# Chrixtar/latentsplat

Hardware: AMD Instinct MI355X
Metric: rendered target views/sec at 256x256, ~300k Gaussians (forward); fwd+bwd ms/view in `fwdbwd` (higher is better)
Workload: dtype f32; 1 GPU; BASELINE configs[1]: 300000 latent Gaussians (4-ch features + opacity), 256x256, forward render; 16 views of one scene per step per GPU; gaussians=300000, parallelism=replicas x1 (one scene per rank, no data-path collective)

## Files before the change

latentsplat_amd/csrc/lsr_key_emit.h:

```cpp
#pragma once
#include "lsr_blend.h"
#include "lsr_tile_scan.h"

namespace lsr {

struct TileRect { int x0, y0, x1, y1; };

__device__ __forceinline__ void count_pairs(uint32_t *hist, int gx, TileRect r, uint32_t span, bool skip_none) {
    if (skip_none) reached_rect(span, r.x0, r.y0, r.x1, r.y1);
    for (int y = r.y0; y < r.y1; ++y)
        for (int x = r.x0; x < r.x1; ++x) atomicAdd(&hist[y * gx + x], 1u);
}

__device__ __forceinline__ void store_bin_record(char *binrec, int narrow, size_t o, bool ok, const TileRect &r, float tz, uint32_t span) {
    const float out_depth = ok ? tz : 0.0f;
    if (narrow) {
        BinRec br;
        br.rect = ok ? ((uint32_t)r.x0 | ((uint32_t)r.y0 << 8) | ((uint32_t)r.x1 << 16) | ((uint32_t)r.y1 << 24)) : 0u;
        br.depth = out_depth; br.span = span;
        ((BinRec *)binrec)[o] = br;
    } else {
        BinRecWide br;
        br.rect = ok ? make_ushort4((unsigned short)r.x0, (unsigned short)r.y0, (unsigned short)r.x1, (unsigned short)r.y1)
                     : make_ushort4(0, 0, 0, 0);
        br.depth = out_depth; br.span = span;
        ((BinRecWide *)binrec)[o] = br;
    }
}

template <int THREADS>
__device__ __forceinline__ void flush_counts(const uint32_t *s_hist, uint32_t *tile_count, int n) {
    __syncthreads();
    for (int t = threadIdx.x; t < n; t += THREADS) {
        const uint32_t c = s_hist[t];
        if (c) atomicAdd(&tile_count[t], c);
    }
}

template <int THREADS>
__device__ __forceinline__ void reserve_segments(const uint32_t *s_hist, uint32_t *s_first, uint32_t *tile_count, int n) {
    __syncthreads();
    for (int t0 = threadIdx.x; t0 < n; t0 += 4 * THREADS) {
        uint32_t c[4], first[4] = {0u, 0u, 0u, 0u};
#pragma unroll
        for (int k = 0; k < 4; ++k) { const int t = t0 + k * THREADS; c[k] = t < n ? s_hist[t] : 0u; }
#pragma unroll
        for (int k = 0; k < 4; ++k) {
            const int t = t0 + k * THREADS;
            if (c[k]) first[k] = __hip_atomic_fetch_add(&tile_count[t], c[k], __ATOMIC_RELAXED, __HIP_MEMORY_SCOPE_AGENT);
        }
#pragma unroll
        for (int k = 0; k < 4; ++k) { const int t = t0 + k * THREADS; if (t < n) s_first[t] = first[k]; }
    }
    __syncthreads();
}

struct KeyBuckets {
    uint32_t *delta;
    uint64_t *key;
    uint32_t *pos;
    uint32_t buf;
    __device__ __forceinline__ KeyBuckets(void *area, size_t bytes, int T) {
        const int kbase = (T * 4 + 7) & ~7;
        delta = (uint32_t *)area;
        key = (uint64_t *)((char *)area + kbase);
        buf = (uint32_t)((bytes - kbase) / 12);
        pos = (uint32_t *)((char *)area + kbase + (size_t)buf * 8);
    }
};

template <int THREADS, int N>
__device__ __forceinline__ void emit_view_keys(uint32_t *cur, const uint32_t *first, const KeyBuckets &kb, const SegOut &seg,
                                               uint32_t seg_view, int T, int gx, bool skip_none,
                                               const uint3 (&br)[N], const int (&index)[N], const bool (&valid)[N]) {
    __shared__ uint32_t s_scanw[THREADS / LSR_WAVE];
    const int tpt = (T + THREADS - 1) / THREADS;
    uint32_t cnt[4], mine = 0;
#pragma unroll
    for (int k = 0; k < 4; ++k) {
        const int t = (int)threadIdx.x * tpt + k;
        cnt[k] = (k < tpt && t < T) ? cur[t] : 0u;
        mine += cnt[k];
    }
    uint32_t n_v;
    uint32_t off = block_exclusive_scan<THREADS>(mine, s_scanw, n_v);
#pragma unroll
    for (int k = 0; k < 4; ++k) {
        const int t = (int)threadIdx.x * tpt + k;
        if (k < tpt && t < T) { cur[t] = off; kb.delta[t] = first[t] - off; off += cnt[k]; }
    }
    __syncthreads();
    const uint32_t cap = seg.cap, seg0 = seg_view * (uint32_t)T;
#pragma unroll
    for (int it = 0; it < N; ++it) {
        const uint32_t rc = valid[it] ? br[it].x : 0u;
        const int x0 = rc & 0xff, y0 = (rc >> 8) & 0xff, x1 = (rc >> 16) & 0xff, y1 = rc >> 24;
        const uint64_t key = ((uint64_t)br[it].y << 32) | ((uint32_t)index[it] << seg.key_shift);
        const uint32_t sp = br[it].z;
        int ex0 = x0, ey0 = y0, ex1 = x1, ey1 = y1;
        if (skip_none) reached_rect(sp, ex0, ey0, ex1, ey1);
        for (int y = ey0; y < ey1; ++y)
            for (int x = ex0; x < ex1; ++x) {
                const int t = y * gx + x;
                const uint32_t code = seg.key_shift ? span_code(sp, x - x0, y - y0) : 0u;
                const uint32_t slot = atomicAdd(&cur[t], 1u);
                const uint32_t pos = (seg0 + (uint32_t)t) * cap + min(slot + kb.delta[t], cap - 1u);
                if (slot < kb.buf) { kb.key[slot] = key | code; kb.pos[slot] = pos; }
                else seg.keys[pos] = key | code;
            }
    }
    __syncthreads();
    const uint32_t nflush = min(n_v, kb.buf);
    for (uint32_t j = threadIdx.x; j < nflush; j += THREADS) seg.keys[kb.pos[j]] = kb.key[j];
    __syncthreads();
}

template <int THREADS>
__device__ __forceinline__ void folded_tile_scan(const FoldedScan &fs, uint32_t *header, const uint32_t *tile_count, int N,
                                                 uint32_t *s_counts, TileScanShared<THREADS> &s_scan) {
    __shared__ uint32_t s_last;
    asm volatile("s_waitcnt vmcnt(0)" ::: "memory");
    __syncthreads();
    if (threadIdx.x == 0) {
        const uint32_t arrived = __hip_atomic_fetch_add(&header[kHdrPreDone], 1u, __ATOMIC_RELAXED, __HIP_MEMORY_SCOPE_AGENT);
        s_last = arrived == gridDim.x * gridDim.y - 1u;
    }
    __syncthreads();
    if (!s_last) return;
    for (int i0 = threadIdx.x; i0 < N; i0 += 4 * THREADS) {
        uint32_t c[4];
#pragma unroll
        for (int k = 0; k < 4; ++k)
            c[k] = __hip_atomic_load(&tile_count[min(i0 + k * THREADS, N - 1)], __ATOMIC_RELAXED, __HIP_MEMORY_SCOPE_AGENT);
#pragma unroll
        for (int k = 0; k < 4; ++k)
            if (i0 + k * THREADS < N) s_counts[i0 + k * THREADS] = c[k];
    }
    __syncthreads();
    tile_scan_block<THREADS, 0, false>(s_counts, fs.tile_start, header, HostMirror{fs.host_words, fs.host_seq},
                                       fs.tile_order, N, fs.capacity, s_scan);
}

}
```

latentsplat_amd/csrc/preprocess.hip:

```cpp
#include <algorithm>

#include "lsr_blend.h"
#include "lsr_depth.h"
#include "lsr_key_emit.h"
#include "lsr_project.h"

namespace lsr {

typedef const float __attribute__((address_space(4))) *kfloat_ptr;

constexpr int kPreThreads = 256;
static_assert(kPreThreads == kPreThreadsScan, "the folded tile scan is sized for this workgroup");
constexpr int kPreItems = 8;

template <int COLOR_MODE, bool LDS_HIST, int VB, bool FMA, bool SEG, bool AA = false>
__global__ void __launch_bounds__(kPreThreads, 6)
k_preprocess(lsr_dims d, lsr_inputs in, float *__restrict__ rec, int RF, char *__restrict__ binrec, int narrow,
             int32_t *__restrict__ radii, uint32_t *__restrict__ tile_count, uint32_t *header, FoldedScan fs, int kItems, SegOut seg) {
    static_assert(!SEG || LDS_HIST, "the key emission reserves its slots from the LDS histogram");
    extern __shared__ uint32_t s_hist[];
    constexpr int kRecRow = kPreThreads + 4;
    __shared__ float4 s_rec[kRecRow * 4];
    static_assert(sizeof(float4) * kRecRow * 4 >= sizeof(uint32_t) * kFoldTiles, "the folded tile scan stages its counts here");
    const bool staged = RF == 16;
    const int v0 = blockIdx.y * VB;
    const int G = d.num_gaussians;
    const int gx = (d.width + LSR_TILE - 1) / LSR_TILE, gy = (d.height + LSR_TILE - 1) / LSR_TILE;
    const int T = gx * gy;
    __shared__ float2 s_focal[VB];
    if (threadIdx.x < VB && v0 + (int)threadIdx.x < d.num_views) {
        const float *vw = in.views + (size_t)(v0 + threadIdx.x) * LSR_VIEW_FLOATS;
        s_focal[threadIdx.x] = make_float2(d.width / (2.0f * vw[35]), d.height / (2.0f * vw[36]));
    }
    if (LDS_HIST)
        for (int t = threadIdx.x; t < VB * T; t += kPreThreads) s_hist[t] = 0;
    __syncthreads();
    const int ce = d.cov_elems;
    const size_t sl = (size_t)input_slice(d, v0);
    const float *means = in.means3D + sl * d.vs_means;
    const float *covs = in.cov3D + sl * d.vs_cov;
    const float *opac = in.opacities + sl * d.vs_opac;
    constexpr int coff = COLOR_MODE == LSR_COLOR_NONE ? 0 : 3;
    const bool direct_feat = d.feat_mode == LSR_FEAT_DIRECT;
    const bool skip_none = reached_only(d);

    const int base = blockIdx.x * (kPreThreads * kItems);
#pragma unroll 1
    for (int it = 0; it < kItems; ++it) {
        const int chunk0 = base + it * kPreThreads;
        if (chunk0 >= G) break;
        const int i = chunk0 + threadIdx.x;
        const bool in_range = i < G;
        const size_t ii = in_range ? (size_t)i : 0;
        const float q0 = means[3 * ii], q1 = means[3 * ii + 1], q2 = means[3 * ii + 2];
        const float *c6 = covs + (size_t)ce * ii;
        const float r0 = c6[0], r1 = c6[1], r2 = c6[2];
        const float r3 = c6[ce == 9 ? 4 : 3], r4 = c6[ce == 9 ? 5 : 4], r5 = c6[ce == 9 ? 8 : 5];
        const float opacity = opac[ii];
        float pay_in[3] = {0.0f, 0.0f, 0.0f};
        if (COLOR_MODE == LSR_COLOR_PRECOMP) {
            const float *cp = in.color + sl * d.vs_color + 3 * ii;
            pay_in[0] = cp[0]; pay_in[1] = cp[1]; pay_in[2] = cp[2];
        }
        const float *fp = in.features + sl * d.vs_feat + ii * d.feat_channels;
        auto payload = [&](int c4) {
            float w[4];
#pragma unroll
            for (int k = 0; k < 4; ++k) {
                const int c = 4 * c4 + k;
                w[k] = c < coff ? pay_in[c < 3 ? c : 0]
                                : ((direct_feat && c - coff < d.feat_channels) ? fp[c - coff] : 0.0f);
            }
            return make_float4(w[0], w[1], w[2], w[3]);
        };
        float4 pay0 = make_float4(0, 0, 0, 0), pay1 = make_float4(0, 0, 0, 0);
        if (staged) { pay0 = payload(0); pay1 = payload(1); }
        asm volatile("" :: "v"(q0), "v"(q1), "v"(q2), "v"(r0), "v"(r1), "v"(r2), "v"(r3), "v"(r4), "v"(r5), "v"(opacity),
                     "v"(pay0.x), "v"(pay0.y), "v"(pay0.z), "v"(pay0.w), "v"(pay1.x), "v"(pay1.y), "v"(pay1.z), "v"(pay1.w));

#pragma unroll 1
        for (int vb = 0; vb < VB; ++vb) {
            const int v = v0 + vb;
            if (v >= d.num_views) break;
            const kfloat_ptr vw = (kfloat_ptr)(in.views + (size_t)v * LSR_VIEW_FLOATS);
            float vm[16], pm[16];
#pragma unroll
            for (int k = 0; k < 16; ++k) { vm[k] = vw[k]; pm[k] = vw[16 + k]; }
            const float tanfovx = vw[35], tanfovy = vw[36];
            const float focal_x = s_focal[vb].x, focal_y = s_focal[vb].y;
            const float limx = 1.3f * tanfovx, limy = 1.3f * tanfovy;
            const float scale = vw[40], scale2 = scale * scale;
            const size_t o = (size_t)v * G + ii;
            const float p0 = q0 * scale, p1 = q1 * scale, p2 = q2 * scale;
            const float s0 = r0 * scale2, s1 = r1 * scale2, s2 = r2 * scale2;
            const float s3 = r3 * scale2, s4 = r4 * scale2, s5 = r5 * scale2;
            const Projected pj = project_gaussian<FMA, AA>(vm, pm, limx, limy, focal_x, focal_y, p0, p1, p2, s0, s1, s2, s3, s4, s5,
                                                       d.width, d.height, gx, gy, in_range);
            const bool ok = pj.ok;
            const float px = pj.px, py = pj.py, conic_a = pj.conic_a, conic_b = pj.conic_b, conic_c = pj.conic_c, tz = pj.tz;
            const float my_radius = pj.radius;
            const float rec_opacity = AA ? opacity * pj.rho : opacity;
            const TileRect rect{pj.rminx, pj.rminy, pj.rmaxx, pj.rmaxy};

            float zpay = tz;
            if (vw[41] != 0.0f) zpay = depth_mode_payload((int)vw[41], tz, scale, vw[42], vw[43]);
            const float4 rr0 = make_float4(px, py, conic_a, conic_b);
            const float4 rr1 = make_float4(conic_c, rec_opacity, ok ? zpay : -1.0f, 0.0f);
            const uint32_t span = ok ? footprint_cells(px, py, conic_a, conic_b, conic_c, rec_opacity, rect.x0, rect.y0) : kSpanNone;
            if (ok) {
                if (!staged) {
                    float4 *R = (float4 *)(rec + o * (size_t)RF);
                    R[0] = rr0; R[1] = rr1;
                    for (int c4 = 0; c4 < (RF - 8) / 4; ++c4) R[2 + c4] = payload(c4);
                }
                count_pairs(LDS_HIST ? s_hist + vb * T : tile_count + (size_t)v * T, gx, rect, span, skip_none);
            }
            if (in_range) {
                radii[o] = ok ? (int32_t)my_radius : 0;
                store_bin_record(binrec, narrow, o, ok, rect, tz, span);
            }
            if (staged) {
                s_rec[0 * kRecRow + threadIdx.x] = rr0;
                s_rec[1 * kRecRow + threadIdx.x] = rr1;
                s_rec[2 * kRecRow + threadIdx.x] = pay0;
                s_rec[3 * kRecRow + threadIdx.x] = pay1;
                __syncthreads();
                float4 *dst = (float4 *)(rec + ((size_t)v * G + chunk0) * 16);
                const int nrec = G - chunk0 < kPreThreads ? G - chunk0 : kPreThreads;
#pragma unroll
                for (int k = 0; k < 4; ++k) {
                    const int idx = k * kPreThreads + threadIdx.x;
                    if (idx < nrec * 4 && s_rec[kRecRow + (idx >> 2)].z >= 0.0f) dst[idx] = s_rec[(idx & 3) * kRecRow + (idx >> 2)];
                }
                __syncthreads();
            }
        }
    }
    const int n_valid = min(VB, d.num_views - v0) * T;
    if (LDS_HIST && !SEG) flush_counts<kPreThreads>(s_hist, tile_count + (size_t)v0 * T, n_valid);
    if (SEG) {
        uint32_t *s_first = s_hist + VB * T;
        reserve_segments<kPreThreads>(s_hist, s_first, tile_count + (size_t)v0 * T, n_valid);
        constexpr int KI = kPreItems / VB;
        const KeyBuckets kb(s_rec, sizeof(s_rec), T);
#pragma unroll 1
        for (int vb = 0; vb < VB; ++vb) {
            const int v = v0 + vb;
            if (v >= d.num_views) break;
            uint3 br[KI];
            int index[KI];
            bool valid[KI];
#pragma unroll
            for (int it = 0; it < KI; ++it) {
                const int i = min(base + min(it, kItems - 1) * kPreThreads + (int)threadIdx.x, G - 1);
                br[it] = *(const uint3 *)(binrec + ((size_t)v * G + (size_t)i) * sizeof(BinRec));
                index[it] = base + it * kPreThreads + (int)threadIdx.x;
                valid[it] = it < kItems && index[it] < G;
            }
            emit_view_keys<kPreThreads, KI>(s_hist + vb * T, s_first + vb * T, kb, seg, (uint32_t)v, T, gx, skip_none, br, index, valid);
        }
    }
    if (fs.enabled) {
        __shared__ TileScanShared<kPreThreads> s_scan;
        folded_tile_scan<kPreThreads>(fs, header, tile_count, d.num_views * T, (uint32_t *)s_rec, s_scan);
    }
}

__global__ void __launch_bounds__(256) k_clear16(uint4 *p, size_t n) {
    for (size_t i = (size_t)blockIdx.x * 256 + threadIdx.x; i < n; i += (size_t)gridDim.x * 256) p[i] = make_uint4(0u, 0u, 0u, 0u);
}
hipError_t launch_clear(void *ptr, size_t bytes, hipStream_t s) {
    const size_t n16 = bytes / 16;
    if (n16 == 0) return hipSuccess;
    const size_t blocks = (n16 + 255) / 256;
    hipLaunchKernelGGL(k_clear16, dim3((unsigned)(blocks < 65536 ? blocks : 65536)), dim3(256), 0, s, (uint4 *)ptr, n16);
    return hipGetLastError();
}

hipError_t launch_preprocess(const lsr_dims &d, const lsr_inputs &in, char *geom, int32_t *radii, const FoldedScan &fs_in,
                             bool seg_mode, hipStream_t s) {
    const GeomLayout L = geom_layout(d);
    const int T = (int)num_tiles(d);
    {
        hipError_t e = launch_clear(geom + L.header, L.tile_start - L.header, s);
        if (e != hipSuccess) return e;
    }
    if (d.num_gaussians == 0) return hipSuccess;
    const bool shared = d.vs_means == 0 && d.vs_cov == 0 && d.vs_opac == 0 && (d.color_mode != LSR_COLOR_PRECOMP || d.vs_color == 0) &&
                        (d.feat_channels == 0 || d.vs_feat == 0);
    const int span = shared ? d.num_views : (d.views_per_group > 1 ? d.views_per_group : 1);
    int vb = (span % 4 == 0 || (shared && span >= 4)) ? 4 : ((span % 2 == 0 || (shared && span >= 2)) ? 2 : 1);
    if (const int forced_vb = env_int("LSR_PRE_VB", 0)) vb = std::min(vb, forced_vb >= 4 ? 4 : (forced_vb >= 2 ? 2 : 1));
    const int64_t yblocks = (d.num_views + vb - 1) / vb;
    const int64_t fill = ((int64_t)d.num_gaussians * yblocks + (int64_t)kPreThreads * 2 * device_cus() - 1) / ((int64_t)kPreThreads * 2 * device_cus());
    const int pre_items = seg_mode ? std::min(kPreItems, std::max(1, env_int("LSR_PRE_ITEMS", kPreItems))) : std::max(1, env_int("LSR_PRE_ITEMS", kPreItems));
    const int items = (int)std::max<int64_t>(1, std::min<int64_t>(std::max(1, pre_items / vb), fill));
    dim3 grid((d.num_gaussians + kPreThreads * items - 1) / (kPreThreads * items), (unsigned)yblocks);
    float *rec = (float *)(geom + L.rec);
    char *binrec = geom + L.bin;
    const int narrow = narrow_bins(d) ? 1 : 0;
    const int RF = L.rec_floats;
    uint32_t *tc = (uint32_t *)(geom + L.tile_count);
    FoldedScan fs = fs_in;
    fs.tile_start = (uint32_t *)(geom + L.tile_start); fs.tile_order = (uint32_t *)(geom + L.tile_order);
    const bool lds = (size_t)T * vb <= 4096;
    const size_t shm = lds ? (size_t)T * vb * 4 * (seg_mode ? 2 : 1) : 0;
    const bool fma = projection_contraction();
    SegOut so{nullptr, 0u, index_packing(d).key_shift};
    if (seg_mode) {
        if (!lds || !narrow || L.seg_cap == 0) return hipErrorInvalidValue;
        so.keys = (uint64_t *)(geom + L.seg_keys); so.cap = L.seg_cap;
    }
    const bool aa = (d.forward_flags & LSR_FWD_ANTIALIAS) != 0;
#define LSR_PRE5(CM, LH, VBV, FM, SG, AAV) hipLaunchKernelGGL((k_preprocess<CM, LH, VBV, FM, SG, AAV>), grid, dim3(kPreThreads), shm, s, d, in, rec, RF, binrec, narrow, radii, tc, (uint32_t *)(geom + L.header), fs, items, so)
#define LSR_PRE4(CM, LH, VBV, FM, SG) do { if (aa) LSR_PRE5(CM, LH, VBV, FM, SG, true); else LSR_PRE5(CM, LH, VBV, FM, SG, false); } while (0)
#define LSR_PRE3(CM, LH, VBV, FM) do { if (LH && seg_mode) LSR_PRE4(CM, LH, VBV, FM, LH); else LSR_PRE4(CM, LH, VBV, FM, false); } while (0)
#define LSR_PRE2(CM, LH, VBV) do { if (fma) LSR_PRE3(CM, LH, VBV, true); else LSR_PRE3(CM, LH, VBV, false); } while (0)
#define LSR_PRE(CM)                                                                              \
    do {                                                                                         \
        if (lds) { if (vb == 4) LSR_PRE2(CM, true, 4); else if (vb == 2) LSR_PRE2(CM, true, 2); else LSR_PRE2(CM, true, 1); } \
        else { if (vb == 4) LSR_PRE2(CM, false, 4); else if (vb == 2) LSR_PRE2(CM, false, 2); else LSR_PRE2(CM, false, 1); } \
    } while (0)
    prof_begin(kStPreprocess, s);
    if (d.color_mode == LSR_COLOR_SH) LSR_PRE(LSR_COLOR_SH);
    else if (d.color_mode == LSR_COLOR_PRECOMP) LSR_PRE(LSR_COLOR_PRECOMP);
    else LSR_PRE(LSR_COLOR_NONE);
#undef LSR_PRE
#undef LSR_PRE2
#undef LSR_PRE3
#undef LSR_PRE4
#undef LSR_PRE5
    prof_end(kStPreprocess, s);
    return hipGetLastError();
}

}
```

latentsplat_amd/csrc/sh.hip:

```cpp
#include <algorithm>
#include <type_traits>

#include "lsr_blend.h"
#include "lsr_depth.h"
#include "lsr_key_emit.h"
#include "lsr_project.h"
#include "lsr_sh.h"

namespace lsr {

constexpr int kShThreads = 256;
constexpr int kShWaves = kShThreads / LSR_WAVE;
constexpr int kShBasisC = 27;
constexpr int kShBasisF = 11;

struct ShParams {
    lsr_dims d;
    lsr_inputs in;
    const float *vis;
    int vis_stride;
    float *rec;
    uint8_t *clamp;
    const float *grec;
    int RF;
// ... 26 lines not shown
__device__ __forceinline__ void stage_group(float *lds, const ShParams &p, int grp, int v, int g0, int rows, int tid) {
    const int ks = p.ks[grp];
    if (!ks) return;
    const int64_t vs = grp == 0 ? p.d.vs_color : p.d.vs_feat;
    const float *src = (grp == 0 ? p.in.color : p.in.features) + (size_t)v * vs + (size_t)g0 * ks;
    float *dst = lds + (grp == 0 ? 0 : p.offF);
    const int n = rows * ks, n4 = (((size_t)src & 15u) == 0) ? n >> 2 : 0;
    const int lane = tid & (LSR_WAVE - 1);
    for (int t4 = tid; t4 - lane < n4; t4 += kShThreads) {
        if (t4 < n4)
            __builtin_amdgcn_global_load_lds((const __attribute__((address_space(1))) void *)(src + 4 * (size_t)t4),
                                             (__attribute__((address_space(3))) void *)(dst + 4 * (size_t)(t4 - lane)), 16, 0, 0);
    }
    for (int t = (n4 << 2) + tid; t < n; t += kShThreads) dst[t] = src[t];
}
__device__ __forceinline__ void staged_barrier() {
    asm volatile("s_waitcnt vmcnt(0)" ::: "memory");
    __syncthreads();
}

template <int MAXDEG, int stride>
__device__ __forceinline__ float sh_dot(const float *bas, const float *co, int deg) {
    float a = bas[0] * co[0];
    if (MAXDEG > 0 && deg > 0) {
#pragma unroll
        for (int k = 1; k < 4; ++k) a += bas[k] * co[k * stride];
        if (MAXDEG > 1 && deg > 1) {
#pragma unroll
            for (int k = 4; k < 9; ++k) a += bas[k] * co[k * stride];
            if (MAXDEG > 2 && deg > 2) {
#pragma unroll
                for (int k = 9; k < 16; ++k) a += bas[k] * co[k * stride];
                if (MAXDEG > 3 && deg > 3) {
#pragma unroll
                    for (int k = 16; k < 25; ++k) a += bas[k] * co[k * stride];
                }
            }
        }
    }
    return a;
}

struct ShDir {
    float dx, dy, dz, len, sc;
};
struct ShPos { float x, y, z; };
typedef const float __attribute__((address_space(4))) *kfloat_ptr;
__device__ __forceinline__ ShPos sh_position(const ShParams &p, int v, int i) {
    const float *mp = p.in.means3D + (size_t)v * p.d.vs_means + 3 * (size_t)i;
    return ShPos{mp[0], mp[1], mp[2]};
}
__device__ __forceinline__ ShDir sh_direction(const ShParams &p, int v, const ShPos &m) {
    const kfloat_ptr vw = (kfloat_ptr)(p.in.views + (size_t)v * LSR_VIEW_FLOATS);
    ShDir r;
    r.sc = vw[40];
    float dx = m.x * r.sc - vw[32], dy = m.y * r.sc - vw[33], dz = m.z * r.sc - vw[34];
    r.len = sqrtf(dx * dx + dy * dy + dz * dz);
    r.dx = dx / r.len; r.dy = dy / r.len; r.dz = dz / r.len;
    return r;
}
__device__ __forceinline__ ShDir sh_direction(const ShParams &p, int v, int i) { return sh_direction(p, v, sh_position(p, v, i)); }

__device__ __forceinline__ bool sh_shared_scene(const ShParams &p) {
    return (!p.has[0] || p.d.vs_color == 0) && (!p.has[1] || p.d.vs_feat == 0);
}

template <int DEGC, int COFF>
__global__ void __launch_bounds__(kShThreads)
k_sh_fwd(ShParams pk) {
    const ShParams p = group_params(pk);
    extern __shared__ float s_lds[];
    const lsr_dims &d = p.d;
    const int tid = threadIdx.x, lane = tid & (LSR_WAVE - 1), wave = __builtin_amdgcn_readfirstlane(tid / LSR_WAVE);
    const int G = d.num_gaussians, V = d.num_views;
    const int g0 = blockIdx.x * LSR_WAVE, i = g0 + lane;
    const int rows = G - g0 < LSR_WAVE ? G - g0 : LSR_WAVE;
    const bool active = i < G;
    const int C = d.feat_channels, K = d.sh_coeffs, Kf = d.feat_sh_coeffs, degF = d.feat_sh_degree;
    const bool hasF = p.has[1] != 0;
    const bool cmaj = d.color_sh_channel_major != 0;
    const bool cax = d.color_sh_convention == LSR_SH_AXES_REFERENCE;
    const float *my = s_lds + lane * p.ks[0];
    const float *myF = s_lds + p.offF + lane * p.ks[1];

    struct Fetched { float visf; ShPos pos; };
    auto fetch = [&](int v) {
        const int vl = v < V ? v : V - 1;
        const size_t o = (size_t)vl * G + (active ? i : 0);
        return Fetched{p.vis[o * p.vis_stride], sh_position(p, vl, active ? i : 0)};
    };
    auto compute = [&](int v, const Fetched &f) {
        const size_t o = (size_t)v * G + (active ? i : 0);
        if (!(active && f.visf > 0.0f)) return;
        const ShDir dir = sh_direction(p, v, f.pos);
        float *R = p.rec + o * (size_t)p.RF + 8;
        float basF[9];
        if (hasF) sh_basis<2>(degF, dir.dz, dir.dx, dir.dy, basF);
        auto feat = [&](int c) -> float {
            if (c >= C) return 0.0f;
            return sh_dot<2, 1>(basF, myF + c * Kf, degF) + 0.5f;
        };
        int c_next = 0;
        if (COFF == 3) {
            float col[3] = {0.0f, 0.0f, 0.0f};
            if (DEGC >= 0) {
                float basC[25];
                sh_basis<DEGC>(DEGC, cax ? dir.dz : dir.dx, cax ? dir.dx : dir.dy, cax ? dir.dy : dir.dz, basC);
                uint32_t bits = 0;
                float a0, a1, a2;
                if (cmaj) {
                    a0 = sh_dot<DEGC, 1>(basC, my, DEGC) + 0.5f;
                    __builtin_amdgcn_sched_barrier(0);
                    a1 = sh_dot<DEGC, 1>(basC, my + K, DEGC) + 0.5f;
                    __builtin_amdgcn_sched_barrier(0);
                    a2 = sh_dot<DEGC, 1>(basC, my + 2 * K, DEGC) + 0.5f;
                } else {
                    a0 = sh_dot<DEGC, 3>(basC, my, DEGC) + 0.5f;
                    __builtin_amdgcn_sched_barrier(0);
                    a1 = sh_dot<DEGC, 3>(basC, my + 1, DEGC) + 0.5f;
                    __builtin_amdgcn_sched_barrier(0);
                    a2 = sh_dot<DEGC, 3>(basC, my + 2, DEGC) + 0.5f;
                }
                if (a0 < 0.0f) bits |= 1u;
                if (a1 < 0.0f) bits |= 2u;
                if (a2 < 0.0f) bits |= 4u;
                col[0] = a0 > 0.0f ? a0 : 0.0f; col[1] = a1 > 0.0f ? a1 : 0.0f; col[2] = a2 > 0.0f ? a2 : 0.0f;
                p.clamp[o] = (uint8_t)bits;
            }
            if (DEGC >= 0 && hasF) {
                *(float4 *)R = make_float4(col[0], col[1], col[2], feat(0));
            } else if (DEGC >= 0) {
                R[0] = col[0]; R[1] = col[1]; R[2] = col[2];
            } else if (hasF) {
                R[3] = feat(0);
            }
            c_next = 1;
        }
        if (hasF) {
            const int pad = ((COFF + C + 3) & ~3) - COFF;
#pragma unroll 1
            for (int c = c_next; c < pad; c += 4)
                *(float4 *)(R + COFF + c) = make_float4(feat(c), feat(c + 1), feat(c + 2), feat(c + 3));
        }
    };

    if (sh_shared_scene(p)) {
        stage_group(s_lds, p, 0, 0, g0, rows, tid);
        stage_group(s_lds, p, 1, 0, g0, rows, tid);
        Fetched f = fetch(wave);
        staged_barrier();
        for (int v = wave; v < V; v += kShWaves) {
            const Fetched nxt = fetch(v + kShWaves);
            compute(v, f);
            f = nxt;
        }
    } else {
        for (int v = 0; v < V; ++v) {
            __syncthreads();
            stage_group(s_lds, p, 0, v, g0, rows, tid);
            stage_group(s_lds, p, 1, v, g0, rows, tid);
            const Fetched f = fetch(v);
            staged_barrier();
            if (wave == (v & (kShWaves - 1))) compute(v, f);
        }
    }
}

struct PreShArgs {
    char *binrec; int narrow;
    int32_t *radii;
    uint32_t *tile_count, *header;
    FoldedScan fs;
    int chunks;
    int lds_hist;
    int hist_off;
    int views_total;
    SegOut seg;
};

#ifndef LSR_PSH_WAVES
#define LSR_PSH_WAVES 1
#endif
template <int DEGC, int COFF, bool FMA, bool SEG, bool AA = false>
__global__ void __launch_bounds__(kShThreads, LSR_PSH_WAVES)
k_preprocess_sh(ShParams pk, PreShArgs a) {
    const ShParams p = group_params(pk);
    extern __shared__ float s_lds[];
    __shared__ float2 s_focal[64];
    const lsr_dims &d = p.d;
    const int tid = threadIdx.x, lane = tid & (LSR_WAVE - 1), wave = __builtin_amdgcn_readfirstlane(tid / LSR_WAVE);
    const int G = d.num_gaussians, V = d.num_views;
    const int gx = (d.width + LSR_TILE - 1) / LSR_TILE, gy = (d.height + LSR_TILE - 1) / LSR_TILE, T = gx * gy;
    const int C = d.feat_channels, K = d.sh_coeffs, Kf = d.feat_sh_coeffs, degF = d.feat_sh_degree;
    const bool hasF = p.has[1] != 0;
    const bool cmaj = d.color_sh_channel_major != 0;
    const bool cax = d.color_sh_convention == LSR_SH_AXES_REFERENCE;
    const int ce = d.cov_elems;
    const int RF = p.RF;
    const bool skip_none = reached_only(d);
    const size_t slot0 = (size_t)blockIdx.y * pk.gs.slots;
    const int view0 = blockIdx.y * (pk.gs.slots ? V : 0);
    int32_t *radii = a.radii + slot0;
    char *binrec = a.binrec + slot0 * (a.narrow ? sizeof(BinRec) : sizeof(BinRecWide));
    uint32_t *tile_count = a.tile_count + (size_t)view0 * T;
    uint32_t *s_hist = (uint32_t *)s_lds + a.hist_off;
    const float *my = s_lds + lane * p.ks[0];
    const float *myF = s_lds + p.offF + lane * p.ks[1];
    for (int v = tid; v < V && v < 64; v += kShThreads) {
        const float *vw = p.in.views + (size_t)v * LSR_VIEW_FLOATS;
        s_focal[v] = make_float2(d.width / (2.0f * vw[35]), d.height / (2.0f * vw[36]));
    }
    if (a.lds_hist)
        for (int t = tid; t < V * T; t += kShThreads) s_hist[t] = 0;

    for (int c = 0; c < a.chunks; ++c) {
        const int g0 = (blockIdx.x * a.chunks + c) * LSR_WAVE;
        if (g0 >= G) break;
        const int i = g0 + lane;
        const int rows = G - g0 < LSR_WAVE ? G - g0 : LSR_WAVE;
        const bool active = i < G;
        const size_t ii = active ? (size_t)i : 0;
        __syncthreads();
        stage_group(s_lds, p, 0, 0, g0, rows, tid);
        stage_group(s_lds, p, 1, 0, g0, rows, tid);
        const float *mp = p.in.means3D + 3 * ii;
        const float q0 = mp[0], q1 = mp[1], q2 = mp[2];
        const float *c6 = p.in.cov3D + (size_t)ce * ii;
        const float r0 = c6[0], r1 = c6[1], r2 = c6[2];
        const float r3 = c6[ce == 9 ? 4 : 3], r4 = c6[ce == 9 ? 5 : 4], r5 = c6[ce == 9 ? 8 : 5];
        const float opacity = p.in.opacities[ii];
        staged_barrier();
        for (int v = wave; v < V; v += kShWaves) {
            const kfloat_ptr vw = (kfloat_ptr)(p.in.views + (size_t)v * LSR_VIEW_FLOATS);
            float vm[16], pm[16];
#pragma unroll
            for (int k = 0; k < 16; ++k) { vm[k] = vw[k]; pm[k] = vw[16 + k]; }
            const float limx = 1.3f * vw[35], limy = 1.3f * vw[36];
            const float2 focal = s_focal[v < 64 ? v : 0];
            const float focal_x = v < 64 ? focal.x : d.width / (2.0f * vw[35]), focal_y = v < 64 ? focal.y : d.height / (2.0f * vw[36]);
            const float scale = vw[40], scale2 = scale * scale;
            const float p0 = q0 * scale, p1 = q1 * scale, p2 = q2 * scale;
            const Projected pj = project_gaussian<FMA, AA>(vm, pm, limx, limy, focal_x, focal_y, p0, p1, p2, r0 * scale2, r1 * scale2, r2 * scale2,
                                                       r3 * scale2, r4 * scale2, r5 * scale2, d.width, d.height, gx, gy, active);
            const bool ok = pj.ok;
            const size_t o = (size_t)v * G + ii;
            const float rec_opacity = AA ? opacity * pj.rho : opacity;
            const uint32_t span = ok ? footprint_cells(pj.px, pj.py, pj.conic_a, pj.conic_b, pj.conic_c, rec_opacity, pj.rminx, pj.rminy) : kSpanNone;
            const TileRect rect{pj.rminx, pj.rminy, pj.rmaxx, pj.rmaxy};
            if (ok) count_pairs(a.lds_hist ? s_hist + v * T : tile_count + (size_t)v * T, gx, rect, span, skip_none);
            if (active) {
                radii[o] = ok ? (int32_t)pj.radius : 0;
                store_bin_record(binrec, a.narrow, o, ok, rect, pj.tz, span);
            }
            if (!ok) continue;
            float zpay = pj.tz;
            if (vw[41] != 0.0f) zpay = depth_mode_payload((int)vw[41], pj.tz, scale, vw[42], vw[43]);
            const ShDir dir = sh_direction(p, v, ShPos{q0, q1, q2});
            float basF[9];
            if (hasF) sh_basis<2>(degF, dir.dz, dir.dx, dir.dy, basF);
            auto feat = [&](int ch) -> float {
                if (ch >= C) return 0.0f;
                return sh_dot<2, 1>(basF, myF + ch * Kf, degF) + 0.5f;
            };
            float col[3] = {0.0f, 0.0f, 0.0f};
            if (DEGC >= 0) {
                float basC[25];
                sh_basis<DEGC>(DEGC, cax ? dir.dz : dir.dx, cax ? dir.dx : dir.dy, cax ? dir.dy : dir.dz, basC);
                uint32_t bits = 0;
                float a0, a1, a2;
                if (cmaj) {
                    a0 = sh_dot<DEGC, 1>(basC, my, DEGC) + 0.5f;
                    __builtin_amdgcn_sched_barrier(0);
                    a1 = sh_dot<DEGC, 1>(basC, my + K, DEGC) + 0.5f;
                    __builtin_amdgcn_sched_barrier(0);
                    a2 = sh_dot<DEGC, 1>(basC, my + 2 * K, DEGC) + 0.5f;
                } else {
                    a0 = sh_dot<DEGC, 3>(basC, my, DEGC) + 0.5f;
                    __builtin_amdgcn_sched_barrier(0);
                    a1 = sh_dot<DEGC, 3>(basC, my + 1, DEGC) + 0.5f;
                    __builtin_amdgcn_sched_barrier(0);
                    a2 = sh_dot<DEGC, 3>(basC, my + 2, DEGC) + 0.5f;
                }
                if (a0 < 0.0f) bits |= 1u;
                if (a1 < 0.0f) bits |= 2u;
                if (a2 < 0.0f) bits |= 4u;
                col[0] = a0 > 0.0f ? a0 : 0.0f; col[1] = a1 > 0.0f ? a1 : 0.0f; col[2] = a2 > 0.0f ? a2 : 0.0f;
                p.clamp[o] = (uint8_t)bits;
            }
            float4 *R = (float4 *)(p.rec + o * (size_t)RF);
            R[0] = make_float4(pj.px, pj.py, pj.conic_a, pj.conic_b);
            R[1] = make_float4(pj.conic_c, rec_opacity, zpay, 0.0f);
            auto slot = [&](int ch) -> float { return ch < COFF ? col[ch < 3 ? ch : 0] : (hasF ? feat(ch - COFF) : 0.0f); };
#pragma unroll 1
            for (int j = 2; j < RF / 4; ++j) {
                const int ch = 4 * (j - 2);
                R[j] = make_float4(slot(ch), slot(ch + 1), slot(ch + 2), slot(ch + 3));
            }
        }
    }
    if (a.lds_hist && !SEG) flush_counts<kShThreads>(s_hist, tile_count, V * T);
    if (SEG) {
        uint32_t *s_first = s_hist + V * T;
        reserve_segments<kShThreads>(s_hist, s_first, tile_count, V * T);
        const KeyBuckets kb(s_lds, (size_t)a.hist_off * 4, T);
#pragma unroll 1
        for (int v = 0; v < V; ++v) {
            uint3 br[2];
            int index[2];
            bool valid[2];
#pragma unroll
            for (int k = 0; k < 2; ++k) {
                const int c = wave + kShWaves * k;
                index[k] = (blockIdx.x * a.chunks + c) * LSR_WAVE + lane;
                valid[k] = c < a.chunks && index[k] < G;
                const int i = min((blockIdx.x * a.chunks + min(c, a.chunks - 1)) * LSR_WAVE + lane, G - 1);
                br[k] = *(const uint3 *)(binrec + ((size_t)v * G + (size_t)i) * sizeof(BinRec));
            }
            emit_view_keys<kShThreads, 2>(s_hist + v * T, s_first + v * T, kb, a.seg, (uint32_t)(view0 + v), T, gx, skip_none, br, index, valid);
        }
    }
    if (a.fs.enabled) {
        TileScanShared<kShThreads> &s_scan = *(TileScanShared<kShThreads> *)((char *)s_lds + (size_t)kFoldTiles * 4);
        folded_tile_scan<kShThreads>(a.fs, a.header, a.tile_count, a.views_total * T, (uint32_t *)s_lds, s_scan);
    }
}

template <int DEGC, int COFF, bool CAM = false>
__global__ void __launch_bounds__(kShThreads, 4)
k_sh_bwd(ShParams pk) {
    const ShParams p = group_params(pk);
    extern __shared__ float s_lds[];
    const lsr_dims &d = p.d;
    const int tid = threadIdx.x, lane = tid & (LSR_WAVE - 1), wave = __builtin_amdgcn_readfirstlane(tid / LSR_WAVE);
    const int G = d.num_gaussians, V = d.num_views;
    const int g0 = blockIdx.x * LSR_WAVE, i = g0 + lane;
    const int rows = G - g0 < LSR_WAVE ? G - g0 : LSR_WAVE;
    const bool active = i < G;
    const int C = d.feat_channels, K = d.sh_coeffs, Kf = d.feat_sh_coeffs, degF = d.feat_sh_degree;
    constexpr int nbC = DEGC >= 0 ? (DEGC + 1) * (DEGC + 1) : 0;
    const int nbF = (degF + 1) * (degF + 1);
    const bool hasF = p.has[1] != 0;
    const bool cmaj = d.color_sh_channel_major != 0;
    const bool cax = d.color_sh_convention == LSR_SH_AXES_REFERENCE;
    const bool shared = sh_shared_scene(p);
    const int chunk = shared ? kShWaves : 1;
    const int ntot = COFF + C, cs = ntot | 1;
    const int area = max(p.offF + LSR_WAVE * p.ks[1], kShWaves * LSR_WAVE * kShBasisC);
    float *s_basC = s_lds, *s_basF = s_lds;
    float *s_gch = s_lds + area;
    const float *my = s_lds + lane * p.ks[0];
    const float *myF = s_lds + p.offF + lane * p.ks[1];
    float acc[3] = {0.0f, 0.0f, 0.0f};

    for (int v0 = 0; v0 < V; v0 += chunk) {
        const int nv = V - v0 < chunk ? V - v0 : chunk;
        __syncthreads();
        stage_group(s_lds, p, 0, shared ? 0 : v0, g0, rows, tid);
        stage_group(s_lds, p, 1, shared ? 0 : v0, g0, rows, tid);
        const int v = v0 + wave;
        const int vl = v < V ? v : V - 1;
        const size_t o = (size_t)vl * G + (active ? i : 0);
        const float visf = p.vis[o * p.vis_stride];
        const uint32_t bits = DEGC >= 0 ? (uint32_t)p.clamp[o] : 0u;
        const ShPos pos = sh_position(p, vl, active ? i : 0);
        const float *gr = p.grec + o * (size_t)p.RF + 8;
        const bool pay8 = ntot <= 8;
        float4 gq0 = make_float4(0.0f, 0.0f, 0.0f, 0.0f), gq1 = gq0;
        if (pay8) { gq0 = *(const float4 *)gr; gq1 = *(const float4 *)(gr + 4); }
        float *mg = s_gch + (wave * LSR_WAVE + lane) * cs;
        staged_barrier();
        const bool vis = wave < nv && active && visf > 0.0f;
        float cq[4] = {0.0f, 0.0f, 0.0f, 0.0f};
        if (pay8) {
            const float gv[8] = {gq0.x, gq0.y, gq0.z, gq0.w, gq1.x, gq1.y, gq1.z, gq1.w};
#pragma unroll
            for (int j = 0; j < 8; ++j)
                if (j < ntot) mg[j] = (vis && !(DEGC >= 0 && j < 3 && (bits >> j & 1u))) ? gv[j] : 0.0f;
        }
        if (vis) {
            const ShDir dir = sh_direction(p, v, pos);
            float ddx = 0.0f, ddy = 0.0f, ddz = 0.0f;
            if (DEGC >= 0) {
                float sg[nbC > 0 ? nbC : 1];
#pragma unroll
                for (int k = 0; k < nbC; ++k) sg[k] = 0.0f;
#pragma unroll 1
                for (int c = 0; c < 3; ++c) {
                    float gc;
                    if (pay8) gc = mg[c];
                    else { gc = (bits >> c & 1u) ? 0.0f : gr[c]; mg[c] = gc; }
                    if (cmaj) {
                        const float *co = my + c * K;
#pragma unroll
                        for (int k = 0; k < nbC; ++k) sg[k] = __builtin_fmaf(co[k], gc, sg[k]);
                    } else {
                        const float *co = my + c;
#pragma unroll
                        for (int k = 0; k < nbC; ++k) sg[k] = __builtin_fmaf(co[3 * k], gc, sg[k]);
                    }
                }
                float dbas[nbC > 0 ? nbC : 1][3];
                sh_basis_grad<DEGC>(DEGC, cax ? dir.dz : dir.dx, cax ? dir.dx : dir.dy, cax ? dir.dy : dir.dz, dbas);
                float c0 = 0.0f, c1 = 0.0f, c2 = 0.0f;
#pragma unroll
                for (int k = 0; k < nbC; ++k) { c0 += dbas[k][0] * sg[k]; c1 += dbas[k][1] * sg[k]; c2 += dbas[k][2] * sg[k]; }
                ddx += cax ? c1 : c0; ddy += cax ? c2 : c1; ddz += cax ? c0 : c2;
            } else if (COFF == 3) {
                mg[0] = mg[1] = mg[2] = 0.0f;
            }
            if (hasF) {
                float sg[9];
#pragma unroll
                for (int k = 0; k < 9; ++k) sg[k] = 0.0f;
#pragma unroll 1
                for (int c = 0; c < C; ++c) {
                    float gc;
                    if (pay8) gc = mg[COFF + c];
                    else { gc = gr[COFF + c]; mg[COFF + c] = gc; }
                    const float *co = myF + c * Kf;
#pragma unroll
                    for (int k = 0; k < 9; ++k)
                        if (k < nbF) sg[k] = __builtin_fmaf(co[k], gc, sg[k]);
                }
                float dbas[9][3];
                sh_basis_grad<2>(degF, dir.dz, dir.dx, dir.dy, dbas);
                float e0 = 0.0f, e1 = 0.0f, e2 = 0.0f;
#pragma unroll
                for (int k = 0; k < 9; ++k)
                    if (k < nbF) { e0 += dbas[k][0] * sg[k]; e1 += dbas[k][1] * sg[k]; e2 += dbas[k][2] * sg[k]; }
                ddx += e1; ddy += e2; ddz += e0;
            } else {
                for (int c = 0; c < C; ++c) mg[COFF + c] = 0.0f;
            }
            const float dot = ddx * dir.dx + ddy * dir.dy + ddz * dir.dz;
            const float f = dir.sc / dir.len;
            const float gm[3] = {(ddx - dir.dx * dot) * f, (ddy - dir.dy * dot) * f, (ddz - dir.dz * dot) * f};
            if constexpr (CAM) {
                const float il = 1.0f / dir.len;
                const float gx = (ddx - dir.dx * dot) * il, gy = (ddy - dir.dy * dot) * il, gz = (ddz - dir.dz * dot) * il;
                cq[0] = -gx; cq[1] = -gy; cq[2] = -gz;
                cq[3] = pos.x * gx + pos.y * gy + pos.z * gz;
            }
            if (d.vs_means != 0) {
                float *o3 = p.g.means3D + (size_t)v * d.vs_means + 3 * (size_t)i;
                o3[0] += gm[0]; o3[1] += gm[1]; o3[2] += gm[2];
            } else {
                acc[0] += gm[0]; acc[1] += gm[1]; acc[2] += gm[2];
            }
        } else {
            for (int j = 0; j < ntot; ++j) mg[j] = 0.0f;
        }
        if constexpr (CAM) {
#pragma unroll
            for (int m = LSR_WAVE / 2; m >= 1; m >>= 1)
#pragma unroll
                for (int k = 0; k < 4; ++k) cq[k] += __shfl_xor(cq[k], m);
            if (lane < 4 && wave < nv) {
                const size_t vg = (size_t)blockIdx.y * V + v;
                p.cam.part[(vg * p.cam.chunks + blockIdx.x) * kCamSlots + kCamPos + lane] =
                    lane == 0 ? cq[0] : (lane == 1 ? cq[1] : (lane == 2 ? cq[2] : cq[3]));
            }
        }
        __syncthreads();
        {
            ShDir dir = {0.0f, 0.0f, 1.0f, 1.0f, 1.0f};
            if (vis) dir = sh_direction(p, v, pos);
            if (DEGC >= 0) {
                float basC[nbC > 0 ? nbC : 1];
                sh_basis<DEGC>(DEGC, cax ? dir.dz : dir.dx, cax ? dir.dx : dir.dy, cax ? dir.dy : dir.dz, basC);
                float *mb = s_basC + (wave * LSR_WAVE + lane) * kShBasisC;
#pragma unroll
                for (int k = 0; k < 26; ++k) mb[k] = (vis && k < nbC) ? basC[k < nbC ? k : 0] : 0.0f;
            }
        }
        __syncthreads();
        const bool rmw_c = d.vs_color == 0 && v0 > 0, rmw_f = d.vs_feat == 0 && v0 > 0;
        if (DEGC >= 0) {
            const int ks = p.ks[0];
            float *dst = p.g.color + (d.vs_color != 0 ? (size_t)v0 * d.vs_color : 0) + (size_t)g0 * ks;
            auto colour_pass = [&](auto RMW) {
                if (ks <= kShThreads) {
                    int t0 = tid;
                    asm volatile("" : "+v"(t0));
                    const int per = udiv_small(kShThreads, p.mdiv[0]);
                    if (t0 >= per * ks) return;
                    const int gq = udiv_small(t0, p.mdiv[0]), rem = t0 - gq * ks;
                    int k, c;
                    if (cmaj) { c = udiv_small(rem, p.mdivK); k = rem - c * K; }
                    else { k = (rem * 0xAAABu) >> 17; c = rem - 3 * k; }
                    const int kb = k < nbC ? k : 25;
                    const float *pb = s_basC + gq * kShBasisC + kb, *pg = s_gch + gq * cs + c;
                    float *o = dst + t0;
                    const int db = per * kShBasisC, dg = per * cs, dd = per * ks;
                    for (int g = gq; g < rows; g += per) {
                        float a = decltype(RMW)::value ? *o : 0.0f;
#pragma unroll
                        for (int vi = 0; vi < kShWaves; ++vi) a = __builtin_fmaf(pb[vi * LSR_WAVE * kShBasisC], pg[vi * LSR_WAVE * cs], a);
                        *o = a;
                        pb += db; pg += dg; o += dd;
                    }
                    return;
                }
                for (int t = tid; t < rows * ks; t += kShThreads) {
                    const int g = udiv_small(t, p.mdiv[0]), rem = t - g * ks;
                    int k, c;
                    if (cmaj) { c = udiv_small(rem, p.mdivK); k = rem - c * K; }
                    else { k = (rem * 0xAAABu) >> 17; c = rem - 3 * k; }
                    const int kb = k < nbC ? k : 25;
                    float a = decltype(RMW)::value ? dst[t] : 0.0f;
                    const float *pb = s_basC + g * kShBasisC + kb, *pg = s_gch + g * cs + c;
#pragma unroll
                    for (int vi = 0; vi < kShWaves; ++vi) a = __builtin_fmaf(pb[vi * LSR_WAVE * kShBasisC], pg[vi * LSR_WAVE * cs], a);
                    dst[t] = a;
                }
            };
            if (rmw_c) colour_pass(std::true_type{}); else colour_pass(std::false_type{});
        }
        if (hasF) {
            if (DEGC >= 0) __syncthreads();
            {
                ShDir dir = {0.0f, 0.0f, 1.0f, 1.0f, 1.0f};
                if (vis) dir = sh_direction(p, v, pos);
                float basF[9];
                sh_basis<2>(degF, dir.dz, dir.dx, dir.dy, basF);
                float *mb = s_basF + (wave * LSR_WAVE + lane) * kShBasisF;
#pragma unroll
                for (int k = 0; k < 9; ++k) mb[k] = (vis && k < nbF) ? basF[k] : 0.0f;
                mb[9] = 0.0f;
            }
            __syncthreads();
            const int ks = p.ks[1];
            float *dst = p.g.features + (d.vs_feat != 0 ? (size_t)v0 * d.vs_feat : 0) + (size_t)g0 * ks;
            auto feature_pass = [&](auto RMW) {
                if (ks <= kShThreads) {
                    int t0 = tid;
                    asm volatile("" : "+v"(t0));
                    const int per = udiv_small(kShThreads, p.mdiv[1]);
                    if (t0 >= per * ks) return;
                    const int gq = udiv_small(t0, p.mdiv[1]), rem = t0 - gq * ks;
                    const int c = udiv_small(rem, p.mdivKf), k = rem - c * Kf;
                    const int kb = k < nbF ? k : 9;
                    const float *pb = s_basF + gq * kShBasisF + kb, *pg = s_gch + gq * cs + COFF + c;
                    float *o = dst + t0;
                    const int db = per * kShBasisF, dg = per * cs, dd = per * ks;
                    for (int g = gq; g < rows; g += per) {
                        float a = decltype(RMW)::value ? *o : 0.0f;
#pragma unroll
                        for (int vi = 0; vi < kShWaves; ++vi) a = __builtin_fmaf(pb[vi * LSR_WAVE * kShBasisF], pg[vi * LSR_WAVE * cs], a);
                        *o = a;
                        pb += db; pg += dg; o += dd;
                    }
                    return;
                }
                for (int t = tid; t < rows * ks; t += kShThreads) {
                    const int g = udiv_small(t, p.mdiv[1]), rem = t - g * ks;
                    const int c = udiv_small(rem, p.mdivKf), k = rem - c * Kf;
                    const int kb = k < nbF ? k : 9;
                    float a = decltype(RMW)::value ? dst[t] : 0.0f;
                    const float *pb = s_basF + g * kShBasisF + kb, *pg = s_gch + g * cs + COFF + c;
#pragma unroll
                    for (int vi = 0; vi < kShWaves; ++vi) a = __builtin_fmaf(pb[vi * LSR_WAVE * kShBasisF], pg[vi * LSR_WAVE * cs], a);
                    dst[t] = a;
                }
            };
            if (rmw_f) feature_pass(std::true_type{}); else feature_pass(std::false_type{});
        }
    }
    if (d.vs_means == 0) {
        __syncthreads();
        float (*s_part)[LSR_WAVE][3] = (float (*)[LSR_WAVE][3])s_lds;
#pragma unroll
        for (int a = 0; a < 3; ++a) s_part[wave][lane][a] = acc[a];
        __syncthreads();
        if (wave == 0 && active) {
            float *o3 = p.g.means3D + 3 * (size_t)i;
#pragma unroll
            for (int a = 0; a < 3; ++a) {
                float t = 0.0f;
#pragma unroll
                for (int w = 0; w < kShWaves; ++w) t += s_part[w][lane][a];
                o3[a] += t;
            }
        }
    }
}

static bool group_enabled(const lsr_dims &d, int group) {
    return group == 0 ? d.color_mode == LSR_COLOR_SH : (d.feat_channels > 0 && d.feat_mode == LSR_FEAT_SH);
}

static uint32_t mdiv_of(int x) { return x > 0 ? (uint32_t)(((1u << 22) + x - 1) / x) : 0u; }

static ShParams make_params(const lsr_dims &d, const lsr_inputs &in, const GeomLayout &L, const char *geom) {
    ShParams p;
    p.d = group_dims(d); p.in = in;
    p.gs = group_strides(d);
    p.vis_stride = (int)(bin_stride(d) / 4);
    p.vis = (const float *)(geom + L.bin) + (narrow_bins(d) ? 1 : 2);
    p.rec = (float *)const_cast<char *>(geom + L.rec);
    p.clamp = (uint8_t *)const_cast<char *>(geom + L.sh_clamp);
    p.grec = nullptr; p.RF = L.rec_floats; p.g = lsr_in_grads{};
    p.has[0] = group_enabled(d, 0); p.has[1] = group_enabled(d, 1);
    p.ks[0] = p.has[0] ? d.sh_coeffs * 3 : 0;
    p.ks[1] = p.has[1] ? d.feat_sh_coeffs * d.feat_channels : 0;
    p.offF = (LSR_WAVE * p.ks[0] + 3) & ~3;
    for (int g = 0; g < 2; ++g) p.mdiv[g] = mdiv_of(p.ks[g]);
    p.mdivK = mdiv_of(d.sh_coeffs); p.mdivKf = mdiv_of(d.feat_sh_coeffs);
// ... 148 lines not shown
```

Measured before the change: 42460 views/s.

## Stage preprocess records per wave and compute all view key offsets in one scan

The staged record write-out now uses a per-wave slice of LDS with a rotated index and wave barriers instead of block-wide __syncthreads, so waves no longer wait on each other for each view. Key emission offsets for all views in a block are computed in a single block scan, folding the per-tile delta into the first array. This removes the separate delta buffer from the key bucket area, which leaves more room for buffered keys. The folded tile scan's shared state now aliases the dynamic histogram LDS, which may raise the dynamic allocation. Risks are correctness of the intra-wave LDS ordering and the multi-view base bookkeeping.

```diff
diff --git a/latentsplat_amd/csrc/lsr_key_emit.h b/latentsplat_amd/csrc/lsr_key_emit.h
--- a/latentsplat_amd/csrc/lsr_key_emit.h
+++ b/latentsplat_amd/csrc/lsr_key_emit.h
@@ -56,40 +56,55 @@
 }
 
 struct KeyBuckets {
-    uint32_t *delta;
     uint64_t *key;
     uint32_t *pos;
     uint32_t buf;
-    __device__ __forceinline__ KeyBuckets(void *area, size_t bytes, int T) {
-        const int kbase = (T * 4 + 7) & ~7;
-        delta = (uint32_t *)area;
-        key = (uint64_t *)((char *)area + kbase);
-        buf = (uint32_t)((bytes - kbase) / 12);
-        pos = (uint32_t *)((char *)area + kbase + (size_t)buf * 8);
+    __device__ __forceinline__ KeyBuckets(void *area, size_t bytes) {
+        key = (uint64_t *)area;
+        buf = (uint32_t)(bytes / 12);
+        pos = (uint32_t *)((char *)area + (size_t)buf * 8);
     }
 };
 
-template <int THREADS, int N>
-__device__ __forceinline__ void emit_view_keys(uint32_t *cur, const uint32_t *first, const KeyBuckets &kb, const SegOut &seg,
-                                               uint32_t seg_view, int T, int gx, bool skip_none,
-                                               const uint3 (&br)[N], const int (&index)[N], const bool (&valid)[N]) {
-    __shared__ uint32_t s_scanw[THREADS / LSR_WAVE];
-    const int tpt = (T + THREADS - 1) / THREADS;
-    uint32_t cnt[4], mine = 0;
+constexpr int kEmitMaxViews = 4;
+
+template <int THREADS, int MAXV>
+__device__ __forceinline__ uint32_t emit_offsets(uint32_t *cur, uint32_t *first, int n, int T, uint32_t *s_wave, uint32_t *s_base) {
+    static_assert(MAXV >= 1 && MAXV <= kEmitMaxViews, "a compare per view and counter");
+    const int per = (n + THREADS - 1) / THREADS;
+    const int lo = min((int)threadIdx.x * per, n), hi = min(lo + per, n);
+    uint32_t mine = 0;
+    for (int t = lo; t < hi; ++t) mine += cur[t];
+    uint32_t total;
+    uint32_t run = block_exclusive_scan<THREADS>(mine, s_wave, total);
+    for (int t = lo; t < hi; ++t) {
+        const uint32_t c = cur[t];
+        if (MAXV == 1) first[t] -= run;
+        else {
 #pragma unroll
-    for (int k = 0; k < 4; ++k) {
-        const int t = (int)threadIdx.x * tpt + k;
-        cnt[k] = (k < tpt && t < T) ? cur[t] : 0u;
-        mine += cnt[k];
+            for (int vb = 0; vb < MAXV; ++vb)
+                if (t == vb * T) s_base[vb] = run;
+        }
+        cur[t] = run; run += c;
     }
-    uint32_t n_v;
-    uint32_t off = block_exclusive_scan<THREADS>(mine, s_scanw, n_v);
+    if (MAXV > 1 && threadIdx.x == 0) s_base[n / T] = total;
+    __syncthreads();
+    if (MAXV == 1) return total;
+    for (int t = threadIdx.x; t < n; t += THREADS) {
+        int vb = 0;
 #pragma unroll
-    for (int k = 0; k < 4; ++k) {
-        const int t = (int)threadIdx.x * tpt + k;
-        if (k < tpt && t < T) { cur[t] = off; kb.delta[t] = first[t] - off; off += cnt[k]; }
+        for (int k = 1; k < MAXV; ++k) vb += t >= k * T ? 1 : 0;
+        const uint32_t c = cur[t] - s_base[vb];
+        cur[t] = c; first[t] -= c;
     }
     __syncthreads();
+    return total;
+}
+
+template <int THREADS, int N>
+__device__ __forceinline__ void emit_view_body(uint32_t *cur, const uint32_t *dfirst, const KeyBuckets &kb, const SegOut &seg,
+                                               uint32_t seg_view, int T, int gx, bool skip_none, uint32_t n_v,
+                                               const uint3 (&br)[N], const int (&index)[N], const bool (&valid)[N]) {
     const uint32_t cap = seg.cap, seg0 = seg_view * (uint32_t)T;
 #pragma unroll
     for (int it = 0; it < N; ++it) {
@@ -104,7 +119,7 @@
                 const int t = y * gx + x;
                 const uint32_t code = seg.key_shift ? span_code(sp, x - x0, y - y0) : 0u;
                 const uint32_t slot = atomicAdd(&cur[t], 1u);
-                const uint32_t pos = (seg0 + (uint32_t)t) * cap + min(slot + kb.delta[t], cap - 1u);
+                const uint32_t pos = (seg0 + (uint32_t)t) * cap + min(slot + dfirst[t], cap - 1u);
                 if (slot < kb.buf) { kb.key[slot] = key | code; kb.pos[slot] = pos; }
                 else seg.keys[pos] = key | code;
             }
@@ -113,6 +128,15 @@
     const uint32_t nflush = min(n_v, kb.buf);
     for (uint32_t j = threadIdx.x; j < nflush; j += THREADS) seg.keys[kb.pos[j]] = kb.key[j];
     __syncthreads();
+}
+
+template <int THREADS, int N>
+__device__ __forceinline__ void emit_view_keys(uint32_t *cur, uint32_t *first, const KeyBuckets &kb, const SegOut &seg,
+                                               uint32_t seg_view, int T, int gx, bool skip_none,
+                                               const uint3 (&br)[N], const int (&index)[N], const bool (&valid)[N]) {
+    __shared__ uint32_t s_scanw[THREADS / LSR_WAVE];
+    const uint32_t n_v = emit_offsets<THREADS, 1>(cur, first, T, T, s_scanw, nullptr);
+    emit_view_body<THREADS, N>(cur, first, kb, seg, seg_view, T, gx, skip_none, n_v, br, index, valid);
 }
 
 template <int THREADS>
diff --git a/latentsplat_amd/csrc/preprocess.hip b/latentsplat_amd/csrc/preprocess.hip
--- a/latentsplat_amd/csrc/preprocess.hip
+++ b/latentsplat_amd/csrc/preprocess.hip
@@ -8,6 +8,11 @@
 namespace lsr {
 
 typedef const float __attribute__((address_space(4))) *kfloat_ptr;
+
+__device__ __forceinline__ void wave_lds_fence() {
+    asm volatile("" ::: "memory");
+    __builtin_amdgcn_wave_barrier();
+}
 
 constexpr int kPreThreads = 256;
 static_assert(kPreThreads == kPreThreadsScan, "the folded tile scan is sized for this workgroup");
@@ -18,10 +23,14 @@
 k_preprocess(lsr_dims d, lsr_inputs in, float *__restrict__ rec, int RF, char *__restrict__ binrec, int narrow,
              int32_t *__restrict__ radii, uint32_t *__restrict__ tile_count, uint32_t *header, FoldedScan fs, int kItems, SegOut seg) {
     static_assert(!SEG || LDS_HIST, "the key emission reserves its slots from the LDS histogram");
-    extern __shared__ uint32_t s_hist[];
+    extern __shared__ __attribute__((aligned(16))) uint32_t s_hist[];
     constexpr int kRecRow = kPreThreads + 4;
     __shared__ float4 s_rec[kRecRow * 4];
     static_assert(sizeof(float4) * kRecRow * 4 >= sizeof(uint32_t) * kFoldTiles, "the folded tile scan stages its counts here");
+    static_assert(kRecRow >= 4 * LSR_WAVE && kPreThreads == 4 * LSR_WAVE, "a slice of four 64-record rows per wave");
+    const int lane = threadIdx.x & (LSR_WAVE - 1), wave = __builtin_amdgcn_readfirstlane(threadIdx.x / LSR_WAVE);
+    float4 *my_rec = s_rec + wave * kRecRow;
+    auto rec_at = [](int k, int r) { return k * LSR_WAVE + ((r + 4 * k) & (LSR_WAVE - 1)); };
     const bool staged = RF == 16;
     const int v0 = blockIdx.y * VB;
     const int G = d.num_gaussians;
@@ -77,6 +86,7 @@
         if (staged) { pay0 = payload(0); pay1 = payload(1); }
         asm volatile("" :: "v"(q0), "v"(q1), "v"(q2), "v"(r0), "v"(r1), "v"(r2), "v"(r3), "v"(r4), "v"(r5), "v"(opacity),
                      "v"(pay0.x), "v"(pay0.y), "v"(pay0.z), "v"(pay0.w), "v"(pay1.x), "v"(pay1.y), "v"(pay1.z), "v"(pay1.w));
+        if (staged) { my_rec[rec_at(2, lane)] = pay0; my_rec[rec_at(3, lane)] = pay1; }
 
 #pragma unroll 1
         for (int vb = 0; vb < VB; ++vb) {
@@ -120,19 +130,17 @@
                 store_bin_record(binrec, narrow, o, ok, rect, tz, span);
             }
             if (staged) {
-                s_rec[0 * kRecRow + threadIdx.x] = rr0;
-                s_rec[1 * kRecRow + threadIdx.x] = rr1;
-                s_rec[2 * kRecRow + threadIdx.x] = pay0;
-                s_rec[3 * kRecRow + threadIdx.x] = pay1;
-                __syncthreads();
-                float4 *dst = (float4 *)(rec + ((size_t)v * G + chunk0) * 16);
-                const int nrec = G - chunk0 < kPreThreads ? G - chunk0 : kPreThreads;
+                my_rec[rec_at(0, lane)] = rr0;
+                my_rec[rec_at(1, lane)] = rr1;
+                wave_lds_fence();
+                float4 *dst = (float4 *)(rec + ((size_t)v * G + chunk0 + wave * LSR_WAVE) * 16);
+                const int nrec = min(G - chunk0 - wave * LSR_WAVE, LSR_WAVE);
 #pragma unroll
                 for (int k = 0; k < 4; ++k) {
-                    const int idx = k * kPreThreads + threadIdx.x;
-                    if (idx < nrec * 4 && s_rec[kRecRow + (idx >> 2)].z >= 0.0f) dst[idx] = s_rec[(idx & 3) * kRecRow + (idx >> 2)];
+                    const int idx = k * LSR_WAVE + lane;
+                    if (idx < nrec * 4 && my_rec[rec_at(1, idx >> 2)].z >= 0.0f) dst[idx] = my_rec[rec_at(idx & 3, idx >> 2)];
                 }
-                __syncthreads();
+                wave_lds_fence();
             }
         }
     }
@@ -142,7 +150,9 @@
         uint32_t *s_first = s_hist + VB * T;
         reserve_segments<kPreThreads>(s_hist, s_first, tile_count + (size_t)v0 * T, n_valid);
         constexpr int KI = kPreItems / VB;
-        const KeyBuckets kb(s_rec, sizeof(s_rec), T);
+        const KeyBuckets kb(s_rec, sizeof(s_rec));
+        __shared__ uint32_t s_scanw[kPreThreads / LSR_WAVE], s_base[VB + 1];
+        const uint32_t n_all = emit_offsets<kPreThreads, VB>(s_hist, s_first, n_valid, T, s_scanw, s_base);
 #pragma unroll 1
         for (int vb = 0; vb < VB; ++vb) {
             const int v = v0 + vb;
@@ -157,11 +167,12 @@
                 index[it] = base + it * kPreThreads + (int)threadIdx.x;
                 valid[it] = it < kItems && index[it] < G;
             }
-            emit_view_keys<kPreThreads, KI>(s_hist + vb * T, s_first + vb * T, kb, seg, (uint32_t)v, T, gx, skip_none, br, index, valid);
+            emit_view_body<kPreThreads, KI>(s_hist + vb * T, s_first + vb * T, kb, seg, (uint32_t)v, T, gx, skip_none,
+                                            VB > 1 ? s_base[vb + 1] - s_base[vb] : n_all, br, index, valid);
         }
     }
     if (fs.enabled) {
-        __shared__ TileScanShared<kPreThreads> s_scan;
+        TileScanShared<kPreThreads> &s_scan = *(TileScanShared<kPreThreads> *)s_hist;
         folded_tile_scan<kPreThreads>(fs, header, tile_count, d.num_views * T, (uint32_t *)s_rec, s_scan);
     }
 }
@@ -204,7 +215,7 @@
     FoldedScan fs = fs_in;
     fs.tile_start = (uint32_t *)(geom + L.tile_start); fs.tile_order = (uint32_t *)(geom + L.tile_order);
     const bool lds = (size_t)T * vb <= 4096;
-    const size_t shm = lds ? (size_t)T * vb * 4 * (seg_mode ? 2 : 1) : 0;
+    const size_t shm = std::max<size_t>(lds ? (size_t)T * vb * 4 * (seg_mode ? 2 : 1) : 0, fs.enabled ? sizeof(TileScanShared<kPreThreads>) : 0);
     const bool fma = projection_contraction();
     SegOut so{nullptr, 0u, index_packing(d).key_shift};
     if (seg_mode) {
diff --git a/latentsplat_amd/csrc/sh.hip b/latentsplat_amd/csrc/sh.hip
--- a/latentsplat_amd/csrc/sh.hip
+++ b/latentsplat_amd/csrc/sh.hip
@@ -352,7 +352,7 @@
     if (SEG) {
         uint32_t *s_first = s_hist + V * T;
         reserve_segments<kShThreads>(s_hist, s_first, tile_count, V * T);
-        const KeyBuckets kb(s_lds, (size_t)a.hist_off * 4, T);
+        const KeyBuckets kb(s_lds, (size_t)a.hist_off * 4);
 #pragma unroll 1
         for (int v = 0; v < V; ++v) {
             uint3 br[2];
```

After: 42510 views/s, median of 3. No clear change (+0.1%).
